# rpng/suo_slam

Measured on AMD Instinct MI355X. Metric: frames/sec (obj-crops/sec) YCB-V 640x480 8-obj; ADD(-S) vs ref, higher is better.
Workload: dtype f32 (2 x fp16 split products)

## Files before the change

suo_slam_amd/csrc/gemm_bf16x3.hip:

```cpp
#include <stdlib.h>
#include <string.h>

#include "buffer_ops.h"
#include "mma_ops.h"
#include "suo_internal.h"
#include "tune.h"

namespace suo {


#ifndef SUO_X3_F16_WAVES
#define SUO_X3_F16_WAVES 3
#endif
#ifndef SUO_X3_BK
#define SUO_X3_BK 16
#endif
constexpr int X3_BN = 128, X3_BK = SUO_X3_BK, X3_GH = X3_BK / 16, X3_PITCH = X3_BK + 8;
constexpr int X3_LPR = X3_BK / 4, X3_RPP = 256 / X3_LPR;
constexpr int X3_ASLOTS = 64 / X3_BK;
#ifndef SUO_X3_BSLOTS
#define SUO_X3_BSLOTS 4
#endif
#ifndef SUO_X3_F16_BSLOTS
#define SUO_X3_F16_BSLOTS 2
#endif
constexpr int X3_BSLOTS = SUO_X3_BSLOTS;
static_assert(X3_BK == 16 || X3_BK == 32, "k-step");

void pack_gemm_weight_bf16x3(const float* W, int N, int K, uint16_t* out) {
    const int NB = N / 32;
    for (int n = 0; n < N; ++n)
        for (int k = 0; k < K; ++k) {
            const int ks = k / 16, kk = k % 16, lane = (kk / 8) * 32 + (n % 32), e = kk % 8, nb = n / 32;
            uint16_t t[3];
            s3_split_host(W[(size_t)n * K + k], t);
            for (int p = 0; p < 3; ++p) out[((((size_t)(ks * NB + nb) * 3 + p) * 64 + lane) * 8) + e] = t[p];
        }
}

void pack_gemm_weight_f16x2(const float* W, int N, int K, uint16_t* out, float* oscale_out) {
    const int NB = N / 32;
    for (int n = 0; n < N; ++n) {
        float mx = 0.f;
        for (int k = 0; k < K; ++k) mx = fmaxf(mx, fabsf(W[(size_t)n * K + k]));
        const int t = s2_row_shift(mx);
        oscale_out[n] = ldexpf(1.f, -(t + S2_XSHIFT));
        for (int k = 0; k < K; ++k) {
            const int ks = k / 16, kk = k % 16, lane = (kk / 8) * 32 + (n % 32), e = kk % 8, nb = n / 32;
            uint16_t h[2];
            s2_split_host(ldexpf(W[(size_t)n * K + k], t), h);
            for (int p = 0; p < 2; ++p) out[((((size_t)(ks * NB + nb) * 2 + p) * 64 + lane) * 8) + e] = h[p];
        }
    }
}


template <bool PRO, bool DUAL, bool RES, bool POOL, int NCB = 2, int RB = 2, int NP = 3>
__global__ __launch_bounds__(256) __attribute__((amdgpu_waves_per_eu(NP == 2 ? SUO_X3_F16_WAVES : 2))) void gemm_bf16x3_kernel(const GemmArgs g, const uint16_t* __restrict__ Wp) {
    static_assert(RB == 2 || !POOL, "the pooled epilogue is laid out for 128-row tiles");
    constexpr int X3_BM = 64 * RB, X3_NR = X3_BM / X3_RPP;
    static_assert(X3_NR >= 1, "64-row tiles need the 16-wide k-step");
    constexpr int PLANE = X3_BM * X3_PITCH;
    constexpr int EPI_BYTES = 4 * 32 * 36 * 4 + (POOL ? 16384 : 0);
    constexpr int SFL = NP * PLANE >= EPI_BYTES / 4 ? NP * PLANE : EPI_BYTES / 4;
    __shared__ __attribute__((aligned(16))) uint16_t S[2][SFL];
    __shared__ __attribute__((aligned(16))) float P[2][512];
    const int tid = threadIdx.x, lane = tid & 63;
    const int w = __builtin_amdgcn_readfirstlane(tid >> 6);
    const int wm = w >> 1, wn = w & 1;
    const int M = g.M, K = g.K1 + (DUAL ? g.K2 : 0), ldo = g.ldo;
    const float xs = NP == 2 ? s2_xscale(g.xscale) : 1.f;
    if (PRO) {
        for (int k = tid; k < g.K1; k += 256) { P[0][k] = NP == 2 ? g.pro_scale[k] * xs : g.pro_scale[k]; P[1][k] = NP == 2 ? g.pro_shift[k] * xs : g.pro_shift[k]; }
    }
    int bid = xcd_block_id();
    static_assert(NCB == 2 || !POOL, "the pooled epilogue is laid out for 128-column tiles");
    constexpr int BN = 64 * NCB;
    const int ntn = g.N / BN, NBT = g.N >> 5;
    const int tn = bid % ntn, mt = bid / ntn, m0 = mt * X3_BM;
    int pool_base = 0;
    if (POOL) {
        const int tpr = g.pool_W >> 6, tpc = (g.pool_H >> 1) * tpr;
        const int l = mt / tpc, rr = mt - l * tpc, yp = rr / tpr, xb = rr - yp * tpr;
        pool_base = (l * g.pool_H + 2 * yp) * g.pool_W + 64 * xb;
    }
    auto pixel_of = [&](int r) -> int { return POOL ? pool_base + (r >> 6) * g.pool_W + (r & 63) : m0 + r; };
    const int ns1 = g.K1 / X3_BK, nsteps = K / X3_BK;
    const __amdgpu_buffer_rsrc_t a1_srd = make_srd(g.A1, (size_t)M * g.lda1 * sizeof(float));
    const __amdgpu_buffer_rsrc_t a2_srd = make_srd(DUAL ? g.A2 : g.A1, DUAL ? (size_t)M * g.lda2 * sizeof(float) : 0);
    const __amdgpu_buffer_rsrc_t w_srd = make_srd(Wp, (size_t)g.N * K * NP * sizeof(uint16_t));
    const int ar = tid / X3_LPR, aq = tid % X3_LPR;
    int avoff1[X3_NR], avoff2[X3_NR];
    bool rok[X3_NR];
#pragma unroll
    for (int i = 0; i < X3_NR; ++i) {
        const int row = pixel_of(X3_RPP * i + ar);
        rok[i] = row < M;
        avoff1[i] = row < M ? (row * g.lda1 + 4 * aq) * 4 : BUF_OOB;
        avoff2[i] = DUAL && row < M ? (row * g.lda2 + 4 * aq) * 4 : BUF_OOB;
    }
    const int wvoff = lane * 16;
    f32x4 araw[X3_ASLOTS][X3_NR];
    constexpr int BSL = NP == 2 ? SUO_X3_F16_BSLOTS : X3_BSLOTS;
    u32x4 braw[BSL][NCB][NP];
    auto requestA = [&](int ks, int slot) {
        if (!DUAL || ks < ns1) {
#pragma unroll
            for (int i = 0; i < X3_NR; ++i) araw[slot][i] = buf_load(a1_srd, avoff1[i], ks * X3_BK * 4);
        } else {
#pragma unroll
            for (int i = 0; i < X3_NR; ++i) araw[slot][i] = buf_load(a2_srd, avoff2[i], (ks - ns1) * X3_BK * 4);
        }
    };
    auto requestB = [&](int kg, int slot) {
#pragma unroll
        for (int cb = 0; cb < NCB; ++cb)
#pragma unroll
            for (int p = 0; p < NP; ++p)
                braw[slot][cb][p] = __builtin_bit_cast(u32x4, buf_load(w_srd, wvoff + p * 1024, ((kg * NBT + 2 * NCB * tn + NCB * wn + cb) * NP) * 1024));
    };
    float xmax = 0.f;
    auto split_store = [&](int ks, int slot, int stage) {
        uint16_t* As = &S[stage][0];
        f32x4 sc, sh;
        if (PRO) { sc = *(const f32x4*)&P[0][ks * X3_BK + 4 * aq]; sh = *(const f32x4*)&P[1][ks * X3_BK + 4 * aq]; }
#pragma unroll
        for (int i = 0; i < X3_NR; ++i) {
            float x[4];
#pragma unroll
            for (int t = 0; t < 4; ++t) x[t] = araw[slot][i][t];
            if (PRO) {
#pragma unroll
                for (int t = 0; t < 4; ++t) x[t] = rok[i] ? fmaxf(fmaf(x[t], sc[t], sh[t]), 0.f) : 0.f;
            }
            if constexpr (NP == 2) {
                if (!PRO) {
#pragma unroll
                    for (int t = 0; t < 4; ++t) x[t] *= xs;
                }
                xmax = s2_track(s2_track(xmax, x[0], x[1]), x[2], x[3]);
            }
            split_store4<NP, PLANE>(&As[(X3_RPP * i + ar) * X3_PITCH + 4 * aq], x[0], x[1], x[2], x[3]);
        }
    };
    f32x16 acc[RB][NCB];
#pragma unroll
    for (int i = 0; i < RB; ++i)
#pragma unroll
        for (int j = 0; j < NCB; ++j)
#pragma unroll
            for (int r = 0; r < 16; ++r) acc[i][j][r] = 0.f;
    const int ngroups = nsteps * X3_GH;
#pragma unroll
    for (int u = 0; u < X3_ASLOTS; ++u) requestA(u < nsteps ? u : nsteps - 1, u);
#pragma unroll
    for (int u = 0; u < BSL; ++u) requestB(u < ngroups ? u : ngroups - 1, u);
    __syncthreads();
    split_store(0, 0, 0);
    const int ko = 8 * (lane >> 5);
    for (int ks0 = 0; ks0 < nsteps; ks0 += X3_ASLOTS) {
#pragma unroll
        for (int u = 0; u < X3_ASLOTS; ++u) {
            const int ks = ks0 + u;
            __syncthreads();
            const uint16_t* As = &S[u & 1][0];
            bf16x8 af[X3_GH][RB][NP];
#pragma unroll
            for (int h = 0; h < X3_GH; ++h)
#pragma unroll
                for (int p = 0; p < NP; ++p)
#pragma unroll
                    for (int rb = 0; rb < RB; ++rb) af[h][rb][p] = *(const bf16x8*)&As[p * PLANE + (32 * RB * wm + 32 * rb + (lane & 31)) * X3_PITCH + ko + 16 * h];
            __builtin_amdgcn_sched_barrier(0);
            if (ks + 1 < nsteps) split_store(ks + 1, (u + 1) % X3_ASLOTS, (u + 1) & 1);
            requestA(ks + X3_ASLOTS < nsteps ? ks + X3_ASLOTS : nsteps - 1, u);
#pragma unroll
            for (int h = 0; h < X3_GH; ++h) {
                const int slot = (u * X3_GH + h) % BSL, kg = ks * X3_GH + h;
                u32x4 bw[NCB][NP];
#pragma unroll
                for (int cb = 0; cb < NCB; ++cb)
#pragma unroll
                    for (int p = 0; p < NP; ++p) bw[cb][p] = braw[slot][cb][p];
                requestB(kg + BSL < ngroups ? kg + BSL : ngroups - 1, slot);
#pragma unroll
                for (int t = 0; t < split_terms<NP>(); ++t)
#pragma unroll
                    for (int rb = 0; rb < RB; ++rb)
#pragma unroll
                        for (int cb = 0; cb < NCB; ++cb) acc[rb][cb] = split_mma<NP>(t, af[h][rb], bw[cb], acc[rb][cb]);
            }
            __builtin_amdgcn_sched_barrier(0);
        }
    }
    __syncthreads();
    if constexpr (NP == 2) s2_raise(g.range_flag, xmax);
    float* T = reinterpret_cast<float*>(&S[0][0]) + w * (32 * 36);
    f32x4* PX = reinterpret_cast<f32x4*>(reinterpret_cast<float*>(&S[0][0]) + 4 * 32 * 36);
    f32x4 hold[POOL ? 2 : 1][POOL ? 2 : 1][POOL ? 4 : 1];
    const __amdgpu_buffer_rsrc_t o_srd = make_srd((POOL && !g.out) ? (float*)g.pool_out : g.out, (POOL && !g.out) ? 0 : (size_t)M * ldo * sizeof(float));
    const __amdgpu_buffer_rsrc_t r_srd = make_srd(RES ? g.R : g.out, RES ? (size_t)M * g.ldr * sizeof(float) : 0);
#pragma unroll
    for (int rb = 0; rb < RB; ++rb)
#pragma unroll
        for (int cb = 0; cb < NCB; ++cb) {
            const int col = BN * tn + 32 * NCB * wn + 32 * cb + (lane & 7) * 4;
            f32x4 bv = f32x4{0.f, 0.f, 0.f, 0.f};
            if (g.bias) bv = *(const f32x4*)(g.bias + col);
            f32x4 osc = f32x4{1.f, 1.f, 1.f, 1.f};
            if constexpr (NP == 2) osc = *(const f32x4*)(g.oscale + col);
            f32x4 rv[RES ? 4 : 1];
            if (RES) {
#pragma unroll
                for (int k = 0; k < 4; ++k) {
                    const int row = pixel_of(32 * RB * wm + 32 * rb + (lane >> 3) + 8 * k);
                    rv[k] = buf_load(r_srd, row < M ? (row * g.ldr + col) * 4 : BUF_OOB, 0);
                }
            }
#pragma unroll
            for (int r = 0; r < 16; ++r) T[patch_at(r, lane)] = acc[rb][cb][r];
            __builtin_amdgcn_wave_barrier();
#pragma unroll
            for (int k = 0; k < 4; ++k) {
                const int row = pixel_of(32 * RB * wm + 32 * rb + (lane >> 3) + 8 * k);
                f32x4 o = patch_row4(T, lane, k);
                if constexpr (NP == 2) o *= osc;
                o += bv;
                if (RES) o += rv[k];
                if (g.relu) {
#pragma unroll
                    for (int q = 0; q < 4; ++q) o[q] = fmaxf(o[q], 0.f);
                }
                if (!POOL || g.out) buf_store(o, o_srd, row < M ? (row * ldo + col) * 4 : BUF_OOB);
                if (POOL) {
                    f32x4 hm;
#pragma unroll
                    for (int q = 0; q < 4; ++q)
                        hm[q] = fmaxf(o[q], __int_as_float(__builtin_amdgcn_mov_dpp(__float_as_int(o[q]), 0x128, 0xf, 0xf, false)));
                    if (wm == 0) hold[rb][cb][k] = hm;
                    else if (!(lane & 8)) PX[(((wn * 2 + rb) * 2 + cb) * 4 + k) * 32 + (lane >> 4) * 8 + (lane & 7)] = hm;
                }
            }
            __builtin_amdgcn_wave_barrier();
        }
    if (POOL) {
        __syncthreads();
        if (wm == 0 && !(lane & 8)) {
            const __amdgpu_buffer_rsrc_t p_srd = make_srd(g.pool_out, (size_t)(M >> 2) * ldo * sizeof(float));
            const int pw = g.pool_W >> 1;
            const int prow0 = (pool_base / g.pool_W >> 1) * pw + ((pool_base % g.pool_W) >> 1);
#pragma unroll
            for (int rb = 0; rb < 2; ++rb)
#pragma unroll
                for (int cb = 0; cb < 2; ++cb)
#pragma unroll
                    for (int k = 0; k < 4; ++k) {
                        const int j = 32 * rb + (lane >> 3) + 8 * k;
                        const int col = 128 * tn + 64 * wn + 32 * cb + (lane & 7) * 4;
                        const f32x4 other = PX[(((wn * 2 + rb) * 2 + cb) * 4 + k) * 32 + (lane >> 4) * 8 + (lane & 7)];
                        f32x4 v;
#pragma unroll
                        for (int q = 0; q < 4; ++q) v[q] = fmaxf(hold[rb][cb][k][q], other[q]);
                        buf_store(v, p_srd, ((prow0 + (j >> 1)) * ldo + col) * 4);
                    }
        }
    }
}

struct GemmChainArgs {
    const float* A; int lda, M;
    const float* bias1; const float* osc1;
    const float* bias2; const float* osc2;
    float* out; int n_valid, hw;
    unsigned* range_flag;
    const float* xs1; const float* xs2;
};

__global__ __launch_bounds__(256) __attribute__((amdgpu_waves_per_eu(3))) void gemm_chain_head_kernel(const GemmChainArgs g, const uint16_t* __restrict__ W1, const uint16_t* __restrict__ W2) {
    static_assert(X3_BK == 16, "written for the 16-wide k-step");
    constexpr int NP = 2, NCB = 2, BM = 64, K1 = 256, N1 = 256, NBT1 = N1 / 32, NB2 = 2;
    constexpr int PLANE = BM * X3_PITCH;
    constexpr int SFL = 4 * 32 * 36 * 4 / 4;
    static_assert(NP * PLANE <= SFL, "stage");
    __shared__ __attribute__((aligned(16))) uint16_t S[2][SFL];
    __shared__ __attribute__((aligned(16))) uint16_t Y[NP][BM * 128];
    const int tid = threadIdx.x, lane = tid & 63;
    const int w = __builtin_amdgcn_readfirstlane(tid >> 6);
    const int wm = w >> 1, wn = w & 1;
    const int M = g.M;
    const float xs1 = s2_xscale(g.xs1), xs2 = s2_xscale(g.xs2);
    int bid = xcd_block_id();
    const int m0 = bid * BM;
    const __amdgpu_buffer_rsrc_t a_srd = make_srd(g.A, (size_t)M * g.lda * sizeof(float));
    const __amdgpu_buffer_rsrc_t w1_srd = make_srd(W1, (size_t)N1 * K1 * NP * sizeof(uint16_t));
    const __amdgpu_buffer_rsrc_t w2_srd = make_srd(W2, (size_t)64 * N1 * NP * sizeof(uint16_t));
    const int ar = tid / X3_LPR, aq = tid % X3_LPR;
    const int arow = m0 + ar;
    const int avoff = arow < M ? (arow * g.lda + 4 * aq) * 4 : BUF_OOB;
    const int wvoff = lane * 16;
    constexpr int BSL = SUO_X3_F16_BSLOTS, nsteps = K1 / X3_BK;
    const int ko = 8 * (lane >> 5);
    float xmax = 0.f;
    f32x16 acc2;
#pragma unroll
    for (int r = 0; r < 16; ++r) acc2[r] = 0.f;
    for (int tn = 0; tn < 2; ++tn) {
        f32x4 araw[X3_ASLOTS];
        u32x4 braw[BSL][NCB][NP];
        auto requestA = [&](int ks, int slot) { araw[slot] = buf_load(a_srd, avoff, ks * X3_BK * 4); };
        auto requestB = [&](int kg, int slot) {
#pragma unroll
            for (int cb = 0; cb < NCB; ++cb)
#pragma unroll
                for (int p = 0; p < NP; ++p)
                    braw[slot][cb][p] = __builtin_bit_cast(u32x4, buf_load(w1_srd, wvoff + p * 1024, ((kg * NBT1 + 2 * NCB * tn + NCB * wn + cb) * NP) * 1024));
        };
        auto split_store = [&](int slot, int stage) {
            uint16_t* As = &S[stage][0];
            float x[4];
#pragma unroll
            for (int t = 0; t < 4; ++t) x[t] = araw[slot][t] * xs1;
            xmax = s2_track(s2_track(xmax, x[0], x[1]), x[2], x[3]);
            split_store4<NP, PLANE>(&As[ar * X3_PITCH + 4 * aq], x[0], x[1], x[2], x[3]);
        };
        f32x16 acc[NCB];
#pragma unroll
        for (int j = 0; j < NCB; ++j)
#pragma unroll
            for (int r = 0; r < 16; ++r) acc[j][r] = 0.f;
#pragma unroll
        for (int u = 0; u < X3_ASLOTS; ++u) requestA(u, u);
#pragma unroll
        for (int u = 0; u < BSL; ++u) requestB(u, u);
        split_store(0, 0);
        for (int ks0 = 0; ks0 < nsteps; ks0 += X3_ASLOTS) {
#pragma unroll
            for (int u = 0; u < X3_ASLOTS; ++u) {
                const int ks = ks0 + u;
                __syncthreads();
                const uint16_t* As = &S[u & 1][0];
                bf16x8 af[NP];
#pragma unroll
                for (int p = 0; p < NP; ++p) af[p] = *(const bf16x8*)&As[p * PLANE + (32 * wm + (lane & 31)) * X3_PITCH + ko];
                __builtin_amdgcn_sched_barrier(0);
                if (ks + 1 < nsteps) split_store((u + 1) % X3_ASLOTS, (u + 1) & 1);
                requestA(ks + X3_ASLOTS < nsteps ? ks + X3_ASLOTS : nsteps - 1, u);
                const int slot = u % BSL;
                u32x4 bw[NCB][NP];
#pragma unroll
                for (int cb = 0; cb < NCB; ++cb)
#pragma unroll
                    for (int p = 0; p < NP; ++p) bw[cb][p] = braw[slot][cb][p];
                requestB(ks + BSL < nsteps ? ks + BSL : nsteps - 1, slot);
#pragma unroll
                for (int t = 0; t < split_terms<NP>(); ++t)
#pragma unroll
                    for (int cb = 0; cb < NCB; ++cb) acc[cb] = split_mma<NP>(t, af, bw[cb], acc[cb]);
                __builtin_amdgcn_sched_barrier(0);
            }
        }
        __syncthreads();
        u32x4 b2[8][NP];
#pragma unroll
        for (int kk = 0; kk < 8; ++kk)
#pragma unroll
            for (int p = 0; p < NP; ++p) b2[kk][p] = __builtin_bit_cast(u32x4, buf_load(w2_srd, wvoff + p * 1024, (((8 * tn + kk) * NB2 + wn) * NP) * 1024));
        float* T = reinterpret_cast<float*>(&S[0][0]) + w * (32 * 36);
#pragma unroll
        for (int cb = 0; cb < NCB; ++cb) {
            const int lcol = 32 * NCB * wn + 32 * cb + (lane & 7) * 4;
            const f32x4 bv = *(const f32x4*)(g.bias1 + 128 * tn + lcol), osc = *(const f32x4*)(g.osc1 + 128 * tn + lcol);
#pragma unroll
            for (int r = 0; r < 16; ++r) T[patch_at(r, lane)] = acc[cb][r];
            __builtin_amdgcn_wave_barrier();
#pragma unroll
            for (int k = 0; k < 4; ++k) {
                const int row = 32 * wm + (lane >> 3) + 8 * k;
                f32x4 o = patch_row4(T, lane, k);
                o *= osc;
                o += bv;
                float y[4];
#pragma unroll
                for (int q = 0; q < 4; ++q) y[q] = fmaxf(o[q], 0.f) * xs2;
                xmax = s2_track(s2_track(xmax, y[0], y[1]), y[2], y[3]);
                split_store4<NP, BM * 128>(&Y[0][row * 128 + (((lcol >> 3) ^ (row & 15)) << 3) + (lcol & 7)], y[0], y[1], y[2], y[3]);
            }
            __builtin_amdgcn_wave_barrier();
        }
        __syncthreads();
        {
            const int yrow = 32 * wm + (lane & 31);
#pragma unroll
            for (int kk = 0; kk < 8; ++kk) {
                const int chunk = (2 * kk + (lane >> 5)) ^ (yrow & 15);
                bf16x8 af[NP];
#pragma unroll
                for (int p = 0; p < NP; ++p) af[p] = *(const bf16x8*)&Y[p][yrow * 128 + chunk * 8];
#pragma unroll
                for (int t = 0; t < split_terms<NP>(); ++t) acc2 = split_mma<NP>(t, af, b2[kk], acc2);
            }
        }
    }
    s2_raise(g.range_flag, xmax);
    const int ch = 32 * wn + (lane & 31);
    if (ch < g.n_valid) {
        const float oc = g.osc2[ch], bb = g.bias2[ch];
        const __amdgpu_buffer_rsrc_t o_srd = make_srd(g.out, (size_t)(M / g.hw) * g.n_valid * g.hw * sizeof(float));
#pragma unroll
        for (int q = 0; q < 4; ++q) {
            const int row = m0 + 32 * wm + 8 * q + 4 * (lane >> 5);
            f32x4 o;
#pragma unroll
            for (int j = 0; j < 4; ++j) o[j] = fmaf(acc2[4 * q + j], oc, bb);
            const int img = row / g.hw, pix = row - img * g.hw;
            buf_store(o, o_srd, row < M ? ((img * g.n_valid + ch) * g.hw + pix) * 4 : BUF_OOB);
        }
    }
}

bool gemm_chain_head_takes(int M, int lda, int n_valid, int hw) {
    return M > 0 && M % 64 == 0 && lda % 4 == 0 && n_valid > 0 && n_valid <= 64 && hw > 0 && hw % 64 == 0 && M % hw == 0 && (size_t)M * lda * 4 < ((size_t)1 << 31);
}

int launch_gemm_chain_head(const float* A, int lda, int M, const uint16_t* W1h, const float* osc1, const float* bias1, const uint16_t* W2h, const float* osc2, const float* bias2,
                           float* out, int n_valid, int hw, unsigned* range_flag, hipStream_t s, const float* xs1, const float* xs2) {
    if (!A || !W1h || !osc1 || !bias1 || !W2h || !osc2 || !bias2 || !out || !range_flag || !gemm_chain_head_takes(M, lda, n_valid, hw)) {
        suo_set_error("gemm_chain_head: unsupported arguments (M=%d lda=%d n_valid=%d hw=%d)", M, lda, n_valid, hw);
        return SUO_ERR_ARG;
    }
    GemmChainArgs g = {A, lda, M, bias1, osc1, bias2, osc2, out, n_valid, hw, range_flag, xs1, xs2};
    hipLaunchKernelGGL(gemm_chain_head_kernel, dim3(M / 64), dim3(256), 0, s, g, W1h, W2h);
    SUO_HIP_CHECK(hipGetLastError());
    return SUO_OK;
}

bool gemm_bf16x3_takes(const GemmArgs& g) {
    const size_t lim = (size_t)1 << 31;
    return g.N > 0 && (g.N % 128 == 0 || (g.N == 64 && !g.pool_out)) && g.n_valid == g.N && g.K1 > 0 && g.K1 % 64 == 0 && g.K2 % 64 == 0 && g.K1 <= 512 && !g.nchw_hw && (g.pool_out ? (g.pool_W % 64 == 0 && g.pool_H % 2 == 0 && g.M % (g.pool_H * g.pool_W) == 0) : g.out != nullptr) &&
           (!g.K2 || (!g.pro_scale && g.A2 && g.lda2 % 4 == 0)) && g.lda1 % 4 == 0 && g.ldo % 4 == 0 && (!g.R || g.ldr % 4 == 0) &&
           ((g.pro_scale == nullptr) == (g.pro_shift == nullptr)) && (size_t)g.M * g.lda1 * 4 < lim && (!g.out || (size_t)g.M * g.ldo * 4 < lim) &&
           (!g.K2 || (size_t)g.M * g.lda2 * 4 < lim) && (!g.R || (size_t)g.M * g.ldr * 4 < lim);
}

template <int NP>
static int launch_gemm_split(const GemmArgs& g, const uint16_t* Wx3, hipStream_t s) {
    if (!gemm_bf16x3_takes(g) || !Wx3 || (NP == 2 && (!g.oscale || !g.range_flag))) {
        suo_set_error("gemm_%s: unsupported shape (N=%d K=%d+%d M=%d)", NP == 3 ? "bf16x3" : "f16x2", g.N, g.K1, g.K2, g.M);
        return SUO_ERR_ARG;
    }
    const bool n64 = g.N % 128 != 0;
    static const long rb1_max_tiles = (long)SUO_TUNE("SUO_X3_ROWS64_MAX_TILES", 1023);
    const long tiles128 = (long)((g.M + 127) / 128) * (n64 ? 1 : g.N / 128);
    const bool rows64 = !n64 && !g.pool_out && X3_BK == 16 && tiles128 <= rb1_max_tiles;
    const int tiles = rows64 ? ((g.M + 63) / 64) * (g.N / 128) : (int)tiles128;
#define X3_LAUNCH(P_, D_, R_) do { if (g.pool_out) hipLaunchKernelGGL((gemm_bf16x3_kernel<P_, D_, R_, true, 2, 2, NP>), dim3(tiles), dim3(256), 0, s, g, Wx3); \
                                   else if (n64) hipLaunchKernelGGL((gemm_bf16x3_kernel<P_, D_, R_, false, 1, 2, NP>), dim3(tiles), dim3(256), 0, s, g, Wx3); \
                                   else if (rows64) hipLaunchKernelGGL((gemm_bf16x3_kernel<P_, D_, R_, false, 2, 1, NP>), dim3(tiles), dim3(256), 0, s, g, Wx3); \
                                   else hipLaunchKernelGGL((gemm_bf16x3_kernel<P_, D_, R_, false, 2, 2, NP>), dim3(tiles), dim3(256), 0, s, g, Wx3); } while (0)
    const bool res = g.R != nullptr;
    if (g.pro_scale) { if (res) X3_LAUNCH(true, false, true); else X3_LAUNCH(true, false, false); }
    else if (g.K2) { if (res) X3_LAUNCH(false, true, true); else X3_LAUNCH(false, true, false); }
    else { if (res) X3_LAUNCH(false, false, true); else X3_LAUNCH(false, false, false); }
#undef X3_LAUNCH
    SUO_HIP_CHECK(hipGetLastError());
    return SUO_OK;
}

int launch_gemm_bf16x3_args(const GemmArgs& g, const uint16_t* Wx3, hipStream_t s) { return launch_gemm_split<3>(g, Wx3, s); }
int launch_gemm_f16x2_args(const GemmArgs& g, const uint16_t* W16, hipStream_t s) { return launch_gemm_split<2>(g, W16, s); }

int launch_gemm_bf16x3(const float* A, int lda, int K, const float* pro_scale, const float* pro_shift, const uint16_t* Wp, const float* bias,
                       float* out, int ldo, int M, int N, int relu, hipStream_t s) {
    GemmArgs g = {};
    g.A1 = A; g.lda1 = lda; g.K1 = K; g.pro_scale = pro_scale; g.pro_shift = pro_shift; g.bias = bias; g.out = out; g.ldo = ldo; g.M = M; g.N = N; g.n_valid = N;
    g.relu = relu;
    return launch_gemm_bf16x3_args(g, Wp, s);
}

}
```

Before: 1371.

## Use a 1x4 wave layout for fp16-split GEMM and chain-head tiles

Adds a W14 variant where each of the four waves covers all 128 tile rows and one 32-column block, instead of the 2x2 layout with 64 rows by 64 columns per wave. Each wave now loads half as much weight data per k-step and reuses it across more rows. It also reads more A fragments from LDS per wave, and the pooled epilogue writes the 2x2 max directly from registers without the shared-memory exchange. It is enabled by default through an env switch for the f16x2 path and the chain-head kernel, and it changes register pressure and the LDS read pattern.

```diff
diff --git a/suo_slam_amd/csrc/gemm_bf16x3.hip b/suo_slam_amd/csrc/gemm_bf16x3.hip
--- a/suo_slam_amd/csrc/gemm_bf16x3.hip
+++ b/suo_slam_amd/csrc/gemm_bf16x3.hip
@@ -55,9 +55,11 @@
 }
 
 
-template <bool PRO, bool DUAL, bool RES, bool POOL, int NCB = 2, int RB = 2, int NP = 3>
+template <bool PRO, bool DUAL, bool RES, bool POOL, int NCB = 2, int RB = 2, int NP = 3, bool W14 = false>
 __global__ __launch_bounds__(256) __attribute__((amdgpu_waves_per_eu(NP == 2 ? SUO_X3_F16_WAVES : 2))) void gemm_bf16x3_kernel(const GemmArgs g, const uint16_t* __restrict__ Wp) {
     static_assert(RB == 2 || !POOL, "the pooled epilogue is laid out for 128-row tiles");
+    static_assert(!W14 || (NP == 2 && NCB == 2 && RB == 2), "the 1 x 4 wave layout is built for the fp16 form's 128 x 128 tiles");
+    constexpr int RBW = W14 ? 2 * RB : RB, NCW = W14 ? NCB / 2 : NCB;
     constexpr int X3_BM = 64 * RB, X3_NR = X3_BM / X3_RPP;
     static_assert(X3_NR >= 1, "64-row tiles need the 16-wide k-step");
     constexpr int PLANE = X3_BM * X3_PITCH;
@@ -67,7 +69,7 @@
     __shared__ __attribute__((aligned(16))) float P[2][512];
     const int tid = threadIdx.x, lane = tid & 63;
     const int w = __builtin_amdgcn_readfirstlane(tid >> 6);
-    const int wm = w >> 1, wn = w & 1;
+    const int wm = W14 ? 0 : w >> 1, wn = W14 ? w : w & 1;
     const int M = g.M, K = g.K1 + (DUAL ? g.K2 : 0), ldo = g.ldo;
     const float xs = NP == 2 ? s2_xscale(g.xscale) : 1.f;
     if (PRO) {
@@ -102,7 +104,7 @@
     const int wvoff = lane * 16;
     f32x4 araw[X3_ASLOTS][X3_NR];
     constexpr int BSL = NP == 2 ? SUO_X3_F16_BSLOTS : X3_BSLOTS;
-    u32x4 braw[BSL][NCB][NP];
+    u32x4 braw[BSL][NCW][NP];
     auto requestA = [&](int ks, int slot) {
         if (!DUAL || ks < ns1) {
 #pragma unroll
@@ -114,10 +116,10 @@
     };
     auto requestB = [&](int kg, int slot) {
 #pragma unroll
-        for (int cb = 0; cb < NCB; ++cb)
+        for (int cb = 0; cb < NCW; ++cb)
 #pragma unroll
             for (int p = 0; p < NP; ++p)
-                braw[slot][cb][p] = __builtin_bit_cast(u32x4, buf_load(w_srd, wvoff + p * 1024, ((kg * NBT + 2 * NCB * tn + NCB * wn + cb) * NP) * 1024));
+                braw[slot][cb][p] = __builtin_bit_cast(u32x4, buf_load(w_srd, wvoff + p * 1024, ((kg * NBT + 2 * NCB * tn + NCW * wn + cb) * NP) * 1024));
     };
     float xmax = 0.f;
     auto split_store = [&](int ks, int slot, int stage) {
@@ -143,11 +145,11 @@
             split_store4<NP, PLANE>(&As[(X3_RPP * i + ar) * X3_PITCH + 4 * aq], x[0], x[1], x[2], x[3]);
         }
     };
-    f32x16 acc[RB][NCB];
-#pragma unroll
-    for (int i = 0; i < RB; ++i)
-#pragma unroll
-        for (int j = 0; j < NCB; ++j)
+    f32x16 acc[RBW][NCW];
+#pragma unroll
+    for (int i = 0; i < RBW; ++i)
+#pragma unroll
+        for (int j = 0; j < NCW; ++j)
 #pragma unroll
             for (int r = 0; r < 16; ++r) acc[i][j][r] = 0.f;
     const int ngroups = nsteps * X3_GH;
@@ -164,31 +166,31 @@
             const int ks = ks0 + u;
             __syncthreads();
             const uint16_t* As = &S[u & 1][0];
-            bf16x8 af[X3_GH][RB][NP];
+            bf16x8 af[X3_GH][RBW][NP];
 #pragma unroll
             for (int h = 0; h < X3_GH; ++h)
 #pragma unroll
                 for (int p = 0; p < NP; ++p)
 #pragma unroll
-                    for (int rb = 0; rb < RB; ++rb) af[h][rb][p] = *(const bf16x8*)&As[p * PLANE + (32 * RB * wm + 32 * rb + (lane & 31)) * X3_PITCH + ko + 16 * h];
+                    for (int rb = 0; rb < RBW; ++rb) af[h][rb][p] = *(const bf16x8*)&As[p * PLANE + (32 * RBW * wm + 32 * rb + (lane & 31)) * X3_PITCH + ko + 16 * h];
             __builtin_amdgcn_sched_barrier(0);
             if (ks + 1 < nsteps) split_store(ks + 1, (u + 1) % X3_ASLOTS, (u + 1) & 1);
             requestA(ks + X3_ASLOTS < nsteps ? ks + X3_ASLOTS : nsteps - 1, u);
 #pragma unroll
             for (int h = 0; h < X3_GH; ++h) {
                 const int slot = (u * X3_GH + h) % BSL, kg = ks * X3_GH + h;
-                u32x4 bw[NCB][NP];
-#pragma unroll
-                for (int cb = 0; cb < NCB; ++cb)
+                u32x4 bw[NCW][NP];
+#pragma unroll
+                for (int cb = 0; cb < NCW; ++cb)
 #pragma unroll
                     for (int p = 0; p < NP; ++p) bw[cb][p] = braw[slot][cb][p];
                 requestB(kg + BSL < ngroups ? kg + BSL : ngroups - 1, slot);
 #pragma unroll
                 for (int t = 0; t < split_terms<NP>(); ++t)
 #pragma unroll
-                    for (int rb = 0; rb < RB; ++rb)
-#pragma unroll
-                        for (int cb = 0; cb < NCB; ++cb) acc[rb][cb] = split_mma<NP>(t, af[h][rb], bw[cb], acc[rb][cb]);
+                    for (int rb = 0; rb < RBW; ++rb)
+#pragma unroll
+                        for (int cb = 0; cb < NCW; ++cb) acc[rb][cb] = split_mma<NP>(t, af[h][rb], bw[cb], acc[rb][cb]);
             }
             __builtin_amdgcn_sched_barrier(0);
         }
@@ -197,14 +199,16 @@
     if constexpr (NP == 2) s2_raise(g.range_flag, xmax);
     float* T = reinterpret_cast<float*>(&S[0][0]) + w * (32 * 36);
     f32x4* PX = reinterpret_cast<f32x4*>(reinterpret_cast<float*>(&S[0][0]) + 4 * 32 * 36);
-    f32x4 hold[POOL ? 2 : 1][POOL ? 2 : 1][POOL ? 4 : 1];
+    f32x4 hold[POOL ? 2 : 1][POOL ? NCW : 1][POOL ? 4 : 1];
+    const __amdgpu_buffer_rsrc_t p14_srd = make_srd(POOL && W14 ? g.pool_out : nullptr, POOL && W14 ? (size_t)(M >> 2) * ldo * sizeof(float) : 0);
+    const int prow14 = POOL && W14 ? (pool_base / g.pool_W >> 1) * (g.pool_W >> 1) + ((pool_base % g.pool_W) >> 1) : 0;
     const __amdgpu_buffer_rsrc_t o_srd = make_srd((POOL && !g.out) ? (float*)g.pool_out : g.out, (POOL && !g.out) ? 0 : (size_t)M * ldo * sizeof(float));
     const __amdgpu_buffer_rsrc_t r_srd = make_srd(RES ? g.R : g.out, RES ? (size_t)M * g.ldr * sizeof(float) : 0);
 #pragma unroll
-    for (int rb = 0; rb < RB; ++rb)
-#pragma unroll
-        for (int cb = 0; cb < NCB; ++cb) {
-            const int col = BN * tn + 32 * NCB * wn + 32 * cb + (lane & 7) * 4;
+    for (int rb = 0; rb < RBW; ++rb)
+#pragma unroll
+        for (int cb = 0; cb < NCW; ++cb) {
+            const int col = BN * tn + 32 * NCW * wn + 32 * cb + (lane & 7) * 4;
             f32x4 bv = f32x4{0.f, 0.f, 0.f, 0.f};
             if (g.bias) bv = *(const f32x4*)(g.bias + col);
             f32x4 osc = f32x4{1.f, 1.f, 1.f, 1.f};
@@ -213,7 +217,7 @@
             if (RES) {
 #pragma unroll
                 for (int k = 0; k < 4; ++k) {
-                    const int row = pixel_of(32 * RB * wm + 32 * rb + (lane >> 3) + 8 * k);
+                    const int row = pixel_of(32 * RBW * wm + 32 * rb + (lane >> 3) + 8 * k);
                     rv[k] = buf_load(r_srd, row < M ? (row * g.ldr + col) * 4 : BUF_OOB, 0);
                 }
             }
@@ -222,7 +226,7 @@
             __builtin_amdgcn_wave_barrier();
 #pragma unroll
             for (int k = 0; k < 4; ++k) {
-                const int row = pixel_of(32 * RB * wm + 32 * rb + (lane >> 3) + 8 * k);
+                const int row = pixel_of(32 * RBW * wm + 32 * rb + (lane >> 3) + 8 * k);
                 f32x4 o = patch_row4(T, lane, k);
                 if constexpr (NP == 2) o *= osc;
                 o += bv;
@@ -237,13 +241,22 @@
 #pragma unroll
                     for (int q = 0; q < 4; ++q)
                         hm[q] = fmaxf(o[q], __int_as_float(__builtin_amdgcn_mov_dpp(__float_as_int(o[q]), 0x128, 0xf, 0xf, false)));
-                    if (wm == 0) hold[rb][cb][k] = hm;
+                    if constexpr (W14) {
+                        if (rb < 2) hold[rb & 1][cb][k] = hm;
+                        else if (!(lane & 8)) {
+                            f32x4 v;
+#pragma unroll
+                            for (int q = 0; q < 4; ++q) v[q] = fmaxf(hold[rb & 1][cb][k][q], hm[q]);
+                            const int j = 32 * (rb & 1) + (lane >> 3) + 8 * k;
+                            buf_store(v, p14_srd, ((prow14 + (j >> 1)) * ldo + col) * 4);
+                        }
+                    } else if (wm == 0) hold[rb][cb][k] = hm;
                     else if (!(lane & 8)) PX[(((wn * 2 + rb) * 2 + cb) * 4 + k) * 32 + (lane >> 4) * 8 + (lane & 7)] = hm;
                 }
             }
             __builtin_amdgcn_wave_barrier();
         }
-    if (POOL) {
+    if (POOL && !W14) {
         __syncthreads();
         if (wm == 0 && !(lane & 8)) {
             const __amdgpu_buffer_rsrc_t p_srd = make_srd(g.pool_out, (size_t)(M >> 2) * ldo * sizeof(float));
@@ -276,6 +289,7 @@
     const float* xs1; const float* xs2;
 };
 
+template <bool W14>
 __global__ __launch_bounds__(256) __attribute__((amdgpu_waves_per_eu(3))) void gemm_chain_head_kernel(const GemmChainArgs g, const uint16_t* __restrict__ W1, const uint16_t* __restrict__ W2) {
     static_assert(X3_BK == 16, "written for the 16-wide k-step");
     constexpr int NP = 2, NCB = 2, BM = 64, K1 = 256, N1 = 256, NBT1 = N1 / 32, NB2 = 2;
@@ -287,6 +301,8 @@
     const int tid = threadIdx.x, lane = tid & 63;
     const int w = __builtin_amdgcn_readfirstlane(tid >> 6);
     const int wm = w >> 1, wn = w & 1;
+    constexpr int RBW = W14 ? 2 : 1, NCW = W14 ? 1 : NCB;
+    const int wm1 = W14 ? 0 : wm, wn1 = W14 ? w : wn;
     const int M = g.M;
     const float xs1 = s2_xscale(g.xs1), xs2 = s2_xscale(g.xs2);
     int bid = xcd_block_id();
@@ -306,14 +322,14 @@
     for (int r = 0; r < 16; ++r) acc2[r] = 0.f;
     for (int tn = 0; tn < 2; ++tn) {
         f32x4 araw[X3_ASLOTS];
-        u32x4 braw[BSL][NCB][NP];
+        u32x4 braw[BSL][NCW][NP];
         auto requestA = [&](int ks, int slot) { araw[slot] = buf_load(a_srd, avoff, ks * X3_BK * 4); };
         auto requestB = [&](int kg, int slot) {
 #pragma unroll
-            for (int cb = 0; cb < NCB; ++cb)
+            for (int cb = 0; cb < NCW; ++cb)
 #pragma unroll
                 for (int p = 0; p < NP; ++p)
-                    braw[slot][cb][p] = __builtin_bit_cast(u32x4, buf_load(w1_srd, wvoff + p * 1024, ((kg * NBT1 + 2 * NCB * tn + NCB * wn + cb) * NP) * 1024));
+                    braw[slot][cb][p] = __builtin_bit_cast(u32x4, buf_load(w1_srd, wvoff + p * 1024, ((kg * NBT1 + 2 * NCB * tn + NCW * wn1 + cb) * NP) * 1024));
         };
         auto split_store = [&](int slot, int stage) {
             uint16_t* As = &S[stage][0];
@@ -323,11 +339,13 @@
             xmax = s2_track(s2_track(xmax, x[0], x[1]), x[2], x[3]);
             split_store4<NP, PLANE>(&As[ar * X3_PITCH + 4 * aq], x[0], x[1], x[2], x[3]);
         };
-        f32x16 acc[NCB];
-#pragma unroll
-        for (int j = 0; j < NCB; ++j)
-#pragma unroll
-            for (int r = 0; r < 16; ++r) acc[j][r] = 0.f;
+        f32x16 acc[RBW][NCW];
+#pragma unroll
+        for (int i = 0; i < RBW; ++i)
+#pragma unroll
+            for (int j = 0; j < NCW; ++j)
+#pragma unroll
+                for (int r = 0; r < 16; ++r) acc[i][j][r] = 0.f;
 #pragma unroll
         for (int u = 0; u < X3_ASLOTS; ++u) requestA(u, u);
 #pragma unroll
@@ -339,23 +357,27 @@
                 const int ks = ks0 + u;
                 __syncthreads();
                 const uint16_t* As = &S[u & 1][0];
-                bf16x8 af[NP];
-#pragma unroll
-                for (int p = 0; p < NP; ++p) af[p] = *(const bf16x8*)&As[p * PLANE + (32 * wm + (lane & 31)) * X3_PITCH + ko];
+                bf16x8 af[RBW][NP];
+#pragma unroll
+                for (int p = 0; p < NP; ++p)
+#pragma unroll
+                    for (int rb = 0; rb < RBW; ++rb) af[rb][p] = *(const bf16x8*)&As[p * PLANE + (32 * RBW * wm1 + 32 * rb + (lane & 31)) * X3_PITCH + ko];
                 __builtin_amdgcn_sched_barrier(0);
                 if (ks + 1 < nsteps) split_store((u + 1) % X3_ASLOTS, (u + 1) & 1);
                 requestA(ks + X3_ASLOTS < nsteps ? ks + X3_ASLOTS : nsteps - 1, u);
                 const int slot = u % BSL;
-                u32x4 bw[NCB][NP];
-#pragma unroll
-                for (int cb = 0; cb < NCB; ++cb)
+                u32x4 bw[NCW][NP];
+#pragma unroll
+                for (int cb = 0; cb < NCW; ++cb)
 #pragma unroll
                     for (int p = 0; p < NP; ++p) bw[cb][p] = braw[slot][cb][p];
                 requestB(ks + BSL < nsteps ? ks + BSL : nsteps - 1, slot);
 #pragma unroll
                 for (int t = 0; t < split_terms<NP>(); ++t)
 #pragma unroll
-                    for (int cb = 0; cb < NCB; ++cb) acc[cb] = split_mma<NP>(t, af, bw[cb], acc[cb]);
+                    for (int rb = 0; rb < RBW; ++rb)
+#pragma unroll
+                        for (int cb = 0; cb < NCW; ++cb) acc[rb][cb] = split_mma<NP>(t, af[rb], bw[cb], acc[rb][cb]);
                 __builtin_amdgcn_sched_barrier(0);
             }
         }
@@ -367,15 +389,17 @@
             for (int p = 0; p < NP; ++p) b2[kk][p] = __builtin_bit_cast(u32x4, buf_load(w2_srd, wvoff + p * 1024, (((8 * tn + kk) * NB2 + wn) * NP) * 1024));
         float* T = reinterpret_cast<float*>(&S[0][0]) + w * (32 * 36);
 #pragma unroll
-        for (int cb = 0; cb < NCB; ++cb) {
-            const int lcol = 32 * NCB * wn + 32 * cb + (lane & 7) * 4;
+        for (int rb = 0; rb < RBW; ++rb)
+#pragma unroll
+        for (int cb = 0; cb < NCW; ++cb) {
+            const int lcol = 32 * NCW * wn1 + 32 * cb + (lane & 7) * 4;
             const f32x4 bv = *(const f32x4*)(g.bias1 + 128 * tn + lcol), osc = *(const f32x4*)(g.osc1 + 128 * tn + lcol);
 #pragma unroll
-            for (int r = 0; r < 16; ++r) T[patch_at(r, lane)] = acc[cb][r];
+            for (int r = 0; r < 16; ++r) T[patch_at(r, lane)] = acc[rb][cb][r];
             __builtin_amdgcn_wave_barrier();
 #pragma unroll
             for (int k = 0; k < 4; ++k) {
-                const int row = 32 * wm + (lane >> 3) + 8 * k;
+                const int row = 32 * RBW * wm1 + 32 * rb + (lane >> 3) + 8 * k;
                 f32x4 o = patch_row4(T, lane, k);
                 o *= osc;
                 o += bv;
@@ -418,6 +442,8 @@
     }
 }
 
+bool gemm_waves_1x4() { return env_switch("SUO_GEMM_WAVES_1X4", 1) != 0; }
+
 bool gemm_chain_head_takes(int M, int lda, int n_valid, int hw) {
     return M > 0 && M % 64 == 0 && lda % 4 == 0 && n_valid > 0 && n_valid <= 64 && hw > 0 && hw % 64 == 0 && M % hw == 0 && (size_t)M * lda * 4 < ((size_t)1 << 31);
 }
@@ -429,7 +455,8 @@
         return SUO_ERR_ARG;
     }
     GemmChainArgs g = {A, lda, M, bias1, osc1, bias2, osc2, out, n_valid, hw, range_flag, xs1, xs2};
-    hipLaunchKernelGGL(gemm_chain_head_kernel, dim3(M / 64), dim3(256), 0, s, g, W1h, W2h);
+    if (gemm_waves_1x4()) hipLaunchKernelGGL(gemm_chain_head_kernel<true>, dim3(M / 64), dim3(256), 0, s, g, W1h, W2h);
+    else hipLaunchKernelGGL(gemm_chain_head_kernel<false>, dim3(M / 64), dim3(256), 0, s, g, W1h, W2h);
     SUO_HIP_CHECK(hipGetLastError());
     return SUO_OK;
 }
@@ -457,11 +484,19 @@
                                    else if (n64) hipLaunchKernelGGL((gemm_bf16x3_kernel<P_, D_, R_, false, 1, 2, NP>), dim3(tiles), dim3(256), 0, s, g, Wx3); \
                                    else if (rows64) hipLaunchKernelGGL((gemm_bf16x3_kernel<P_, D_, R_, false, 2, 1, NP>), dim3(tiles), dim3(256), 0, s, g, Wx3); \
                                    else hipLaunchKernelGGL((gemm_bf16x3_kernel<P_, D_, R_, false, 2, 2, NP>), dim3(tiles), dim3(256), 0, s, g, Wx3); } while (0)
+#define X3_LAUNCH14(P_, D_, R_) do { if constexpr (NP == 2) { if (g.pool_out) hipLaunchKernelGGL((gemm_bf16x3_kernel<P_, D_, R_, true, 2, 2, 2, true>), dim3(tiles), dim3(256), 0, s, g, Wx3); \
+                                     else hipLaunchKernelGGL((gemm_bf16x3_kernel<P_, D_, R_, false, 2, 2, 2, true>), dim3(tiles), dim3(256), 0, s, g, Wx3); } } while (0)
     const bool res = g.R != nullptr;
-    if (g.pro_scale) { if (res) X3_LAUNCH(true, false, true); else X3_LAUNCH(true, false, false); }
+    if (NP == 2 && !n64 && !rows64 && gemm_waves_1x4()) {
+        if (g.pro_scale) { if (res) X3_LAUNCH14(true, false, true); else X3_LAUNCH14(true, false, false); }
+        else if (g.K2) { if (res) X3_LAUNCH14(false, true, true); else X3_LAUNCH14(false, true, false); }
+        else { if (res) X3_LAUNCH14(false, false, true); else X3_LAUNCH14(false, false, false); }
+    }
+    else if (g.pro_scale) { if (res) X3_LAUNCH(true, false, true); else X3_LAUNCH(true, false, false); }
     else if (g.K2) { if (res) X3_LAUNCH(false, true, true); else X3_LAUNCH(false, true, false); }
     else { if (res) X3_LAUNCH(false, false, true); else X3_LAUNCH(false, false, false); }
 #undef X3_LAUNCH
+#undef X3_LAUNCH14
     SUO_HIP_CHECK(hipGetLastError());
     return SUO_OK;
 }
```

New measurement: 1388, median of 6. +1.2%, better.
